# tencent-ailab/pika

Hardware: NVIDIA H100
Metric: utterances/sec RNN-T train step (T=1000,U=150,V=6k) (higher is better)
Workload: dtype bf16

## Files before the change

### pika_b200/csrc/gemm.cu

```cuda
#include <cstdarg>
#include <cstdio>
#include <cstdlib>
#include <cstring>

#include "../../include/pika_b200.h"
#include "common.cuh"

namespace pk {

constexpr int BM = 128;
constexpr int BK = 64;
constexpr int A_STAGE_BYTES = BM * BK * 2;
constexpr int C_STAGE_BYTES = 64 * 128;
constexpr int CONSUMERS = 2;

struct GemmParams {
    CUtensorMap a[PK_GEMM_MAX_PAIRS];
    CUtensorMap b[PK_GEMM_MAX_PAIRS];
    CUtensorMap c;
    int a_off[PK_GEMM_MAX_PAIRS];
    int b_off[PK_GEMM_MAX_PAIRS];
    int n_pairs, kz_count, num_k_blocks;
    int k_splits, iters_per_split;
    int split_major;
    int M, N, tiles_m, tiles_n, zb0, zb1;
    int a_sel2, a_sel3, b_sel2, b_sel3;
    int c_is_f32, c_accumulate;
    float alpha;
    const float* bias;
    int act;
    uint32_t drop_thresh;
    float drop_scale;
    uint32_t drop_seed;
    int aux_mode, aux_is_f32;
    const void* aux;
    long long aux_sm, aux_s0, aux_s1;
    float aux_scale;
    float* row_lse;
    uint64_t pol_a, pol_b, pol_c;
};

template <int BN, bool TWO, bool EPI_WARPS> struct GemmCfg {
    static constexpr int B_STAGE_BYTES = BN * BK * 2;
    static constexpr int STAGE_BYTES = A_STAGE_BYTES + B_STAGE_BYTES;
    static constexpr int STAGES = BN == 256 ? (EPI_WARPS ? 3 : 4) : (BN == 128 ? 6 : 8);
    static constexpr int C_OFF = STAGES * STAGE_BYTES;
    static constexpr int C_BYTES = EPI_WARPS ? BM * BN * 2 : CONSUMERS * 2 * C_STAGE_BYTES;
    static constexpr int BIAS_OFF = C_OFF + C_BYTES;
    static constexpr int BAR_OFF = BIAS_OFF + (EPI_WARPS ? BN * 4 : 0);
    static constexpr int SMEM_BYTES = BAR_OFF + 256 + 1024;
    static constexpr int THREADS = 128 + CONSUMERS * 128;
    static constexpr int RELEASES = CONSUMERS * (TWO ? 2 : 1);
    static_assert(!TWO || BN == 256, "the CTA-pair kernel works on 256 x 256 tiles");
    static_assert(SMEM_BYTES <= 232448, "shared memory budget");
};

PK_DEVICE int pick_sel(int sel, int zb0, int zb1, int kz) {
    return sel == PK_SEL_ZB0 ? zb0 : (sel == PK_SEL_ZB1 ? zb1 : (sel == PK_SEL_KZ ? kz : 0));
}

struct UnitCoord { int mb, nb, zb0, zb1, split; };
PK_DEVICE UnitCoord decode_unit(const GemmParams& p, int unit, int out_tiles) {
    UnitCoord u;
    int tile;
    if (p.split_major) { u.split = unit / out_tiles; tile = unit - u.split * out_tiles; }
    else { tile = unit / p.k_splits; u.split = unit - tile * p.k_splits; }
    const int tiles_per_z = p.tiles_m * p.tiles_n;
    const int z = tile / tiles_per_z;
    const int r = tile - z * tiles_per_z;
    u.mb = r / p.tiles_n; u.nb = r - u.mb * p.tiles_n;
    u.zb1 = z / p.zb0; u.zb0 = z - u.zb1 * p.zb0;
    return u;
}

template <int BN, bool A_MN, bool B_MN> PK_DEVICE void wgmma_tile(float (&acc)[BN / 2], uint64_t a, uint64_t b, uint32_t accumulate) {
    if constexpr (BN == 64) wgmma_ss_n64<A_MN, B_MN>(acc, a, b, accumulate);
    else if constexpr (BN == 128) wgmma_ss_n128<A_MN, B_MN>(acc, a, b, accumulate);
    else wgmma_ss_n256<A_MN, B_MN>(acc, a, b, accumulate);
}

enum { EPI_PLAIN = 0, EPI_LSE = 1, EPI_FULL = 2 };
template <bool CF32, int EPI> constexpr bool epi_warps() { return !CF32 && EPI != EPI_FULL; }

template <bool A_MN, bool B_MN, int BN, bool CF32, int EPI, bool TWO>
__global__ void __launch_bounds__(GemmCfg<BN, TWO, epi_warps<CF32, EPI>()>::THREADS, 1) gemm_wgmma_kernel(const __grid_constant__ GemmParams p) {
    constexpr bool EW = epi_warps<CF32, EPI>();
    static_assert(EPI != EPI_LSE || (EW && BN == 256), "the row log-sum-exp epilogue works on bf16 256-wide tiles");
    using Cfg = GemmCfg<BN, TWO, EW>;
    extern __shared__ uint8_t smem_raw[];
    uint8_t* smem = reinterpret_cast<uint8_t*>((reinterpret_cast<uintptr_t>(smem_raw) + 1023) & ~uintptr_t(1023));
    uint64_t* full_bar = reinterpret_cast<uint64_t*>(smem + Cfg::BAR_OFF);
    uint64_t* empty_bar = full_bar + Cfg::STAGES;
    uint64_t* c_full = empty_bar + Cfg::STAGES;
    uint64_t* c_empty = c_full + 1;
    const uint32_t ctile = smem_u32(smem + Cfg::C_OFF);
    const uint32_t sbias = smem_u32(smem + Cfg::BIAS_OFF);

    const int warp = threadIdx.x >> 5;
    const int lane = threadIdx.x & 31;
    const uint32_t rank = TWO ? cluster_ctarank() : 0u;
    const int worker = TWO ? (int)(blockIdx.x >> 1) : (int)blockIdx.x;
    const int n_workers = TWO ? (int)(gridDim.x >> 1) : (int)gridDim.x;

    if (threadIdx.x == 0) {
        for (int i = 0; i < p.n_pairs; ++i) {
            tma_prefetch_desc(&p.a[i]);
            tma_prefetch_desc(&p.b[i]);
        }
        tma_prefetch_desc(&p.c);
        for (int s = 0; s < Cfg::STAGES; ++s) {
            mbar_init(&full_bar[s], 1);
            mbar_init(&empty_bar[s], Cfg::RELEASES);
        }
        if (EW) {
            mbar_init(c_full, CONSUMERS * 4);
            mbar_init(c_empty, 3);
        }
        mbar_fence_init();
    }
    if (TWO) cluster_sync_all(); else __syncthreads();

    const int out_tiles = p.tiles_m * p.tiles_n * p.zb0 * p.zb1;
    const int num_units = out_tiles * p.k_splits;
    const int k_iters_total = p.n_pairs * p.kz_count * p.num_k_blocks;

    if (warp < 4) {
        setmaxnreg_dec<40>();
    }
    if (warp == 0) {
        const uint32_t lead = elect_one_u32();
        int stage = 0;
        uint32_t phase = 0;
        const int kzb = p.kz_count * p.num_k_blocks;
        for (int unit = worker; unit < num_units; unit += n_workers) {
            const UnitCoord u = decode_unit(p, unit, out_tiles);
            const int m0 = TWO ? u.mb * (2 * BM) + (int)rank * BM : u.mb * BM, n0 = u.nb * BN;
            const int i0 = u.split * p.iters_per_split, i1 = min(k_iters_total, i0 + p.iters_per_split);
            int pr = i0 / kzb;
            int rem = i0 - pr * kzb;
            int kz = rem / p.num_k_blocks, kb = rem - kz * p.num_k_blocks;
            int a2 = pick_sel(p.a_sel2, u.zb0, u.zb1, kz), a3 = pick_sel(p.a_sel3, u.zb0, u.zb1, kz);
            int b2 = pick_sel(p.b_sel2, u.zb0, u.zb1, kz), b3 = pick_sel(p.b_sel3, u.zb0, u.zb1, kz);
            const CUtensorMap* ma = &p.a[pr];
            const CUtensorMap* mbp = &p.b[pr];
            int a_off = p.a_off[pr], b_off = p.b_off[pr];
            for (int i = i0; i < i1; ++i) {
                mbar_wait(&empty_bar[stage], phase ^ 1);
                uint8_t* sa = smem + stage * Cfg::STAGE_BYTES;
                uint8_t* sb = sa + A_STAGE_BYTES;
                mbar_arrive_expect_tx_p(&full_bar[stage], Cfg::STAGE_BYTES, lead);
                const int k0 = kb * BK;
                if (A_MN) {
#pragma unroll
                    for (int c = 0; c < BM / 64; ++c)
                        tma_load_4d_hint_p(sa + c * (64 * BK * 2), ma, &full_bar[stage], m0 + c * 64, k0 + a_off, a2, a3, p.pol_a, lead);
                } else {
                    tma_load_4d_hint_p(sa, ma, &full_bar[stage], k0, m0 + a_off, a2, a3, p.pol_a, lead);
                }
                if (TWO) {
                    if (B_MN) {
#pragma unroll
                        for (int c = 0; c < BN / 128; ++c) {
                            const int cc = (int)rank * (BN / 128) + c;
                            tma_load_4d_mc_hint_p(sb + cc * (64 * BK * 2), mbp, &full_bar[stage], n0 + cc * 64, k0 + b_off, b2, b3, 3, p.pol_b, lead);
                        }
                    } else {
                        tma_load_4d_mc_hint_p(sb + (int)rank * (BN / 2) * 128, mbp, &full_bar[stage], k0, n0 + (int)rank * (BN / 2) + b_off, b2, b3, 3,
                                              p.pol_b, lead);
                    }
                } else if (B_MN) {
#pragma unroll
                    for (int c = 0; c < BN / 64; ++c)
                        tma_load_4d_hint_p(sb + c * (64 * BK * 2), mbp, &full_bar[stage], n0 + c * 64, k0 + b_off, b2, b3, p.pol_b, lead);
                } else {
                    tma_load_4d_hint_p(sb, mbp, &full_bar[stage], k0, n0 + b_off, b2, b3, p.pol_b, lead);
                }
                if (++stage == Cfg::STAGES) { stage = 0; phase ^= 1; }
                if (++kb == p.num_k_blocks) {
                    kb = 0;
                    if (++kz == p.kz_count) {
                        kz = 0;
                        if (++pr < p.n_pairs) { ma = &p.a[pr]; mbp = &p.b[pr]; a_off = p.a_off[pr]; b_off = p.b_off[pr]; }
                    }
                    a2 = pick_sel(p.a_sel2, u.zb0, u.zb1, kz); a3 = pick_sel(p.a_sel3, u.zb0, u.zb1, kz);
                    b2 = pick_sel(p.b_sel2, u.zb0, u.zb1, kz); b3 = pick_sel(p.b_sel3, u.zb0, u.zb1, kz);
                }
            }
        }
    }
    if (EW && warp >= 1 && warp < 4) {
        const int et = threadIdx.x - 32;
        const uint32_t store_pred = (threadIdx.x == 32) ? 1u : 0u;
        uint32_t cph = 0;
        for (int unit = worker; unit < num_units; unit += n_workers, cph ^= 1) {
            const UnitCoord u = decode_unit(p, unit, out_tiles);
            const int m0 = TWO ? u.mb * (2 * BM) + (int)rank * BM : u.mb * BM, n0 = u.nb * BN;
            for (int c = et; c < BN; c += 96) sts_f32(sbias + c * 4, (p.bias != nullptr && n0 + c < p.N) ? __ldg(p.bias + n0 + c) : 0.f);
            __syncwarp();
            if (lane == 0) mbar_arrive(c_empty);
            mbar_wait(c_full, cph);
#pragma unroll
            for (int ch = 0; ch < BN / 64; ++ch)
#pragma unroll
                for (int h = 0; h < 2; ++h)
                    if (n0 + ch * 64 < p.N && m0 + h * 64 < p.M)
                        tma_store_4d_hint_p(&p.c, smem + Cfg::C_OFF + ch * (BM * 128) + h * (64 * 128), n0 + ch * 64, m0 + h * 64, u.zb0, u.zb1,
                                            p.pol_c, store_pred);
            tma_store_commit_p(store_pred);
            if constexpr (EPI == EPI_LSE) {
                constexpr float L2E = 1.4426950408889634f;
                const int half = lane & 1;
                const int nvalid = p.N - n0 - half * 128;
                const int rot = half * 4;
                for (int r = (et >> 5) * 16 + (lane >> 1); r < BM; r += 48) {
                    const uint32_t rowa = ctile + half * (2 * BM * 128) + r * 128;
                    uint32_t mx[4] = {0xFF80FF80u, 0xFF80FF80u, 0xFF80FF80u, 0xFF80FF80u};
#pragma unroll
                    for (int j = 0; j < 16; ++j) {
                        const int g = (j & 7) ^ rot;
                        if ((j >> 3) * 64 + g * 8 < nvalid) {
                            const uint4 v = lds_u32x4(rowa + (j >> 3) * (BM * 128) + ((g ^ (r & 7)) << 4));
                            mx[0] = bf16x2_max(mx[0], v.x); mx[1] = bf16x2_max(mx[1], v.y);
                            mx[2] = bf16x2_max(mx[2], v.z); mx[3] = bf16x2_max(mx[3], v.w);
                        }
                    }
                    const uint32_t m2 = bf16x2_max(bf16x2_max(mx[0], mx[1]), bf16x2_max(mx[2], mx[3]));
                    const float m = fmaxf(bf16lo(m2), bf16hi(m2)) * L2E;
                    float s[4] = {0.f, 0.f, 0.f, 0.f};
#pragma unroll
                    for (int j = 0; j < 16; ++j) {
                        const int g = (j & 7) ^ rot;
                        if ((j >> 3) * 64 + g * 8 < nvalid) {
                            const uint4 v = lds_u32x4(rowa + (j >> 3) * (BM * 128) + ((g ^ (r & 7)) << 4));
                            const uint32_t w[4] = {v.x, v.y, v.z, v.w};
#pragma unroll
                            for (int q = 0; q < 4; ++q)
                                s[q] += ex2_approx(fmaf(bf16lo(w[q]), L2E, -m)) + ex2_approx(fmaf(bf16hi(w[q]), L2E, -m));
                        }
                    }
                    const float sum = (s[0] + s[1]) + (s[2] + s[3]);
                    const float mo = __shfl_xor_sync(0xffffffffu, m, 1);
                    const float so = __shfl_xor_sync(0xffffffffu, sum, 1);
                    const float mm = fmaxf(m, mo);
                    const float st = (mm == -INFINITY) ? 0.f : sum * ex2_approx(m - mm) + so * ex2_approx(mo - mm);
                    if (half == 0 && m0 + r < p.M)
                        *reinterpret_cast<float2*>(p.row_lse + ((size_t)u.nb * (size_t)p.M + (size_t)(m0 + r)) * 2) = make_float2(mm, st);
                }
            }
            tma_store_wait_read_p<0>(store_pred);
        }
        if (store_pred) tma_store_wait<0>();
    }
    if (warp >= 4) {
    setmaxnreg_inc<232>();
    const int wg = (threadIdx.x >> 7) - 1;
    const int et = threadIdx.x & 127;
    const int w4 = et >> 5;
    const uint32_t store_pred = (et == 0) ? 1u : 0u;
    const int bar_stage = 1 + wg;
    constexpr int GW = CF32 ? 4 : 8;
    constexpr int CH = 8 * GW;
    constexpr int ES = CF32 ? 4 : 2;
    uint8_t* cst = smem + Cfg::C_OFF + wg * 2 * C_STAGE_BYTES;
    const float relu_floor = (p.act == PK_ACT_RELU) ? 0.f : -INFINITY;
    const uint32_t base16 = (smem_u32(smem) >> 4) & 0x3FFF;
    const uint64_t a_desc0 = (A_MN ? make_smem_desc_sw128(0, 64 * BK * 2, 1024) : make_smem_desc_sw128(0, 16, 1024)) + base16 + ((wg * 8192) >> 4);
    const uint64_t b_desc0 = (B_MN ? make_smem_desc_sw128(0, 64 * BK * 2, 1024) : make_smem_desc_sw128(0, 16, 1024)) + base16 + (A_STAGE_BYTES >> 4);
    constexpr uint32_t A_K16 = (A_MN ? 2048 : 32) >> 4, B_K16 = (B_MN ? 2048 : 32) >> 4;
    const int r0 = w4 * 16 + (lane >> 2);
    const int cq = (lane & 3) * 2;

    float acc[BN / 2];
    int stage = 0;
    uint32_t phase = 0;
    uint32_t chunk_ctr = 0;
    uint32_t cph = 0;
    auto release = [&](int s) {
        if (et == 0) { mbar_arrive(&empty_bar[s]); if (TWO) mbar_arrive_remote(&empty_bar[s], rank ^ 1u); }
    };
    for (int unit = worker; unit < num_units; unit += n_workers) {
        const UnitCoord u = decode_unit(p, unit, out_tiles);
        const int k_iters = min(k_iters_total, (u.split + 1) * p.iters_per_split) - u.split * p.iters_per_split;
        int prev = -1;
        for (int k = 0; k < k_iters; ++k) {
            mbar_wait(&full_bar[stage], phase);
            const uint32_t st16 = (uint32_t)(stage * Cfg::STAGE_BYTES) >> 4;
            wgmma_fence_acc(acc);
            wgmma_fence();
#pragma unroll
            for (int k4 = 0; k4 < BK / 16; ++k4)
                wgmma_tile<BN, A_MN, B_MN>(acc, a_desc0 + st16 + k4 * A_K16, b_desc0 + st16 + k4 * B_K16, (k > 0 || k4 > 0) ? 1u : 0u);
            wgmma_commit();
            wgmma_fence_acc(acc);
            wgmma_wait<1>();
            if (prev >= 0) release(prev);
            prev = stage;
            if (++stage == Cfg::STAGES) { stage = 0; phase ^= 1; }
        }
        wgmma_wait<0>();
        wgmma_fence_acc(acc);
        if (prev >= 0) release(prev);

        if constexpr (EW) {
            mbar_wait(c_empty, cph);
            const int mi = lane >> 3;
            const uint32_t row_addr = ctile + (uint32_t)(wg * 64 + w4 * 16 + (lane & 7) + ((mi & 1) << 3)) * 128;
#pragma unroll
            for (int q = 0; q < BN / 16; ++q) {
                uint32_t r[4];
#pragma unroll
                for (int i = 0; i < 2; ++i) {
                    const int blk = 2 * q + i;
                    const float2 bs = lds_f32x2(sbias + (blk * 8 + cq) * 4);
#pragma unroll
                    for (int h = 0; h < 2; ++h)
                        r[2 * i + h] = pack_bf16x2(fmaxf(fmaf(acc[blk * 4 + 2 * h], p.alpha, bs.x), relu_floor),
                                                   fmaxf(fmaf(acc[blk * 4 + 2 * h + 1], p.alpha, bs.y), relu_floor));
                }
                const int blk = 2 * q + (mi >> 1);
                stmatrix_x4(row_addr + (blk >> 3) * (BM * 128) + (((blk & 7) ^ (lane & 7)) << 4), r[0], r[1], r[2], r[3]);
            }
            fence_proxy_async_smem();
            __syncwarp();
            if (lane == 0) mbar_arrive(c_full);
            cph ^= 1;
            continue;
        }

        const int zb0 = u.zb0, zb1 = u.zb1;
        const int m0 = (TWO ? u.mb * (2 * BM) + (int)rank * BM : u.mb * BM) + wg * 64;
        const int n0 = u.nb * BN;
        if (m0 >= p.M) continue;
        const int mrow[2] = {m0 + r0, m0 + r0 + 8};
        const unsigned char* aux_row[2] = {nullptr, nullptr};
        uint64_t lin_row[2];
#pragma unroll
        for (int h = 0; h < 2; ++h) {
            if (EPI == EPI_FULL && p.aux_mode != PK_AUX_NONE && mrow[h] < p.M) {
                const long long off = (long long)mrow[h] * p.aux_sm + (long long)zb0 * p.aux_s0 + (long long)zb1 * p.aux_s1;
                aux_row[h] = reinterpret_cast<const unsigned char*>(p.aux) + off * (p.aux_is_f32 ? 4 : 2);
            }
            lin_row[h] = ((uint64_t)(zb1 * p.zb0 + zb0) * (uint64_t)p.M + (uint64_t)mrow[h]) * (uint64_t)p.N;
        }
        constexpr int n_chunks = BN / CH;
#pragma unroll
        for (int ch = 0; ch < n_chunks; ++ch) {
            const int nc0 = n0 + ch * CH;
            if (nc0 >= p.N) break;
            uint8_t* sbuf = cst + (chunk_ctr & 1) * C_STAGE_BYTES;
            tma_store_wait_read_p<1>(store_pred);
            named_bar_sync(bar_stage, 128);
#pragma unroll
            for (int nb = 0; nb < CH / 8; ++nb) {
                const int cl = nb * 8 + cq;
                const int ncol = nc0 + cl;
                float bs[2];
                if (p.bias != nullptr && ncol < p.N) { bs[0] = __ldg(p.bias + ncol); bs[1] = (ncol + 1 < p.N) ? __ldg(p.bias + ncol + 1) : 0.f; }
                else { bs[0] = 0.f; bs[1] = 0.f; }
#pragma unroll
                for (int h = 0; h < 2; ++h) {
                    const int ai = (ch * (CH / 8) + nb) * 4 + 2 * h;
                    float x[2];
#pragma unroll
                    for (int e = 0; e < 2; ++e) x[e] = fmaxf(fmaf(acc[ai + e], p.alpha, bs[e]), relu_floor);
                    if (EPI == EPI_FULL && p.drop_thresh != 0u) {
#pragma unroll
                        for (int e = 0; e < 2; ++e)
                            x[e] = drop_keep(lin_row[h] + (uint64_t)(ncol + e), p.drop_seed, p.drop_thresh) ? x[e] * p.drop_scale : 0.f;
                    }
                    if (EPI == EPI_FULL && aux_row[h] != nullptr && ncol < p.N) {
                        float a[2];
                        if (p.aux_is_f32) {
                            const float2 t2 = *reinterpret_cast<const float2*>(aux_row[h] + (size_t)ncol * 4);
                            a[0] = t2.x; a[1] = t2.y;
                        } else {
                            const uint32_t t1 = *reinterpret_cast<const uint32_t*>(aux_row[h] + (size_t)ncol * 2);
                            a[0] = bf16lo(t1); a[1] = bf16hi(t1);
                        }
                        if (p.aux_mode == PK_AUX_ADD) { x[0] += a[0]; x[1] += a[1]; }
                        else { x[0] = (a[0] != 0.f) ? x[0] * p.aux_scale : 0.f; x[1] = (a[1] != 0.f) ? x[1] * p.aux_scale : 0.f; }
                    }
                    const int row = r0 + 8 * h;
                    const int boff = cl * ES;
                    uint8_t* dst = sbuf + row * 128 + ((((boff >> 4) ^ (row & 7))) << 4) + (boff & 15);
                    if (CF32) {
                        *reinterpret_cast<float2*>(dst) = make_float2(x[0], x[1]);
                    } else {
                        *reinterpret_cast<uint32_t*>(dst) = pack_bf16x2(x[0], x[1]);
                    }
                }
            }
            fence_proxy_async_smem();
            named_bar_sync(bar_stage, 128);
            if (p.c_accumulate) tma_reduce_add_4d_p(&p.c, sbuf, nc0, m0, zb0, zb1, store_pred);
            else tma_store_4d_hint_p(&p.c, sbuf, nc0, m0, zb0, zb1, p.pol_c, store_pred);
            tma_store_commit_p(store_pred);
            ++chunk_ctr;
        }
    }
    if (!EW && store_pred) tma_store_wait<0>();
    }
    if (TWO) cluster_sync_all();
}

typedef CUresult (*EncodeTiledFn)(CUtensorMap*, CUtensorMapDataType, cuuint32_t, void*, const cuuint64_t*,
                                  const cuuint64_t*, const cuuint32_t*, const cuuint32_t*, CUtensorMapInterleave,
                                  CUtensorMapSwizzle, CUtensorMapL2promotion, CUtensorMapFloatOOBfill);

static EncodeTiledFn get_encode_fn() {
    static EncodeTiledFn fn = nullptr;
    if (fn) return fn;
    void* ptr = nullptr;
    cudaDriverEntryPointQueryResult qres;
    cudaError_t e = cudaGetDriverEntryPoint("cuTensorMapEncodeTiled", &ptr, cudaEnableDefault, &qres);
    if (e != cudaSuccess || qres != cudaDriverEntryPointSuccess || ptr == nullptr) return nullptr;
    fn = reinterpret_cast<EncodeTiledFn>(ptr);
    return fn;
}

static int make_map(CUtensorMap* out, const pk_view4& v, int is_f32, int box0, int box1, const char* what) {
    EncodeTiledFn enc = get_encode_fn();
    if (!enc) { set_last_error("cuTensorMapEncodeTiled entry point not available"); return -3; }
    const int es = is_f32 ? 4 : 2;
    cuuint64_t dims[4];
    cuuint64_t strides[3];
    cuuint32_t box[4] = {(cuuint32_t)box0, (cuuint32_t)box1, 1, 1};
    cuuint32_t estr[4] = {1, 1, 1, 1};
    for (int i = 0; i < 4; ++i) {
        if (v.dim[i] <= 0) { set_last_error("gemm %s: dim[%d]=%lld must be > 0", what, i, (long long)v.dim[i]); return -1; }
        dims[i] = (cuuint64_t)v.dim[i];
    }
    for (int i = 0; i < 3; ++i) {
        long long sb = (long long)v.stride[i] * es;
        if (v.dim[i + 1] == 1 && (sb <= 0 || (sb % 16) != 0)) sb = 16;
        if (sb <= 0 || (sb % 16) != 0) {
            set_last_error("gemm %s: stride[%d]=%lld elements is not a positive multiple of 16 bytes", what, i,
                           (long long)v.stride[i]);
            return -1;
        }
        strides[i] = (cuuint64_t)sb;
    }
    if ((reinterpret_cast<uintptr_t>(v.ptr) & 15) != 0) { set_last_error("gemm %s: base pointer not 16B aligned", what); return -1; }
    if ((cuuint64_t)box[1] > 256) { set_last_error("gemm %s: box too large", what); return -1; }
    CUresult r = enc(out, is_f32 ? CU_TENSOR_MAP_DATA_TYPE_FLOAT32 : CU_TENSOR_MAP_DATA_TYPE_BFLOAT16, 4,
                     const_cast<void*>(v.ptr), dims, strides, box, estr, CU_TENSOR_MAP_INTERLEAVE_NONE,
                     CU_TENSOR_MAP_SWIZZLE_128B, CU_TENSOR_MAP_L2_PROMOTION_L2_256B, CU_TENSOR_MAP_FLOAT_OOB_FILL_NONE);
    if (r != CUDA_SUCCESS) { set_last_error("gemm %s: cuTensorMapEncodeTiled failed with CUresult %d", what, (int)r); return -3; }
    return 0;
}

void count_launch();

int encode_tiled_bf16_3d(CUtensorMap* out, const void* ptr, const unsigned long long (&dims)[3], const unsigned long long (&strides_bytes)[2],
                         const unsigned (&box)[3], const char* what) {
    EncodeTiledFn enc = get_encode_fn();
    if (!enc) { set_last_error("cuTensorMapEncodeTiled entry point not available"); return -3; }
    {
        static thread_local bool ctx_ready = false;
        if (!ctx_ready) { PK_CHECK_CUDA(cudaFree(nullptr)); ctx_ready = true; }
    }
    cuuint64_t d[3] = {dims[0], dims[1], dims[2]};
    cuuint64_t st[2] = {strides_bytes[0], strides_bytes[1]};
    cuuint32_t bx[3] = {box[0], box[1], box[2]};
    cuuint32_t es[3] = {1, 1, 1};
    if ((reinterpret_cast<uintptr_t>(ptr) & 15) != 0 || (st[0] % 16) != 0 || (st[1] % 16) != 0) {
        set_last_error("%s: base pointer / strides must be 16-byte aligned", what);
        return -1;
    }
    CUresult r = enc(out, CU_TENSOR_MAP_DATA_TYPE_BFLOAT16, 3, const_cast<void*>(ptr), d, st, bx, es, CU_TENSOR_MAP_INTERLEAVE_NONE,
                     CU_TENSOR_MAP_SWIZZLE_128B, CU_TENSOR_MAP_L2_PROMOTION_L2_256B, CU_TENSOR_MAP_FLOAT_OOB_FILL_NONE);
    if (r != CUDA_SUCCESS) { set_last_error("%s: cuTensorMapEncodeTiled failed with CUresult %d", what, (int)r); return -3; }
    return 0;
}

template <bool A_MN, bool B_MN, int BN, bool CF32, int EPI, bool TWO>
static int launch_gemm_e(const GemmParams& gp, int workers, cudaStream_t stream) {
    using Cfg = GemmCfg<BN, TWO, epi_warps<CF32, EPI>()>;
    auto kern = gemm_wgmma_kernel<A_MN, B_MN, BN, CF32, EPI, TWO>;
    static bool configured = false;
    if (!configured) {
        PK_CHECK_CUDA(cudaFuncSetAttribute(kern, cudaFuncAttributeMaxDynamicSharedMemorySize, Cfg::SMEM_BYTES));
        configured = true;
    }
    if (TWO) {
        cudaLaunchConfig_t cfg = {};
        cfg.gridDim = dim3(2 * workers);
        cfg.blockDim = dim3(Cfg::THREADS);
        cfg.dynamicSmemBytes = Cfg::SMEM_BYTES;
        cfg.stream = stream;
        cudaLaunchAttribute attr[1];
        attr[0].id = cudaLaunchAttributeClusterDimension;
        attr[0].val.clusterDim.x = 2; attr[0].val.clusterDim.y = 1; attr[0].val.clusterDim.z = 1;
        cfg.attrs = attr;
        cfg.numAttrs = 1;
        static int max_pairs = -1;
        if (max_pairs < 0) {
            int n = 0;
            PK_CHECK_CUDA(cudaOccupancyMaxActiveClusters(&n, kern, &cfg));
            PK_CHECK_ARG(n > 0, "gemm: no 2-CTA cluster of the pair kernel fits on this device");
            max_pairs = n;
        }
        if (workers > max_pairs) {
            workers = max_pairs;
            cfg.gridDim = dim3(2 * workers);
        }
        PK_CHECK_CUDA(cudaLaunchKernelEx(&cfg, kern, gp));
    } else {
        kern<<<workers, Cfg::THREADS, Cfg::SMEM_BYTES, stream>>>(gp);
        PK_CHECK_LAUNCH();
    }
    count_launch();
    return 0;
}

template <bool A_MN, bool B_MN, int BN, bool CF32, bool TWO>
static int launch_gemm(const GemmParams& gp, int workers, cudaStream_t stream) {
    if (gp.row_lse != nullptr) {
        if constexpr (!A_MN && !B_MN && BN == 256 && !CF32) return launch_gemm_e<false, false, 256, false, EPI_LSE, TWO>(gp, workers, stream);
        set_last_error("gemm: row_lse needs K-major operands, a bf16 C and block_n = 256");
        return -1;
    }
    if (gp.drop_thresh != 0u || gp.aux_mode != PK_AUX_NONE) return launch_gemm_e<A_MN, B_MN, BN, CF32, EPI_FULL, TWO>(gp, workers, stream);
    return launch_gemm_e<A_MN, B_MN, BN, CF32, EPI_PLAIN, TWO>(gp, workers, stream);
}

template <int BN, bool TWO>
static int dispatch_major(const GemmParams& gp, int a_mn, int b_mn, int workers, cudaStream_t stream) {
    if (gp.c_is_f32) {
        if (!a_mn && !b_mn) return launch_gemm<false, false, BN, true, TWO>(gp, workers, stream);
        if (!a_mn && b_mn) return launch_gemm<false, true, BN, true, TWO>(gp, workers, stream);
        if (a_mn && !b_mn) return launch_gemm<true, false, BN, true, TWO>(gp, workers, stream);
        return launch_gemm<true, true, BN, true, TWO>(gp, workers, stream);
    }
    if (!a_mn && !b_mn) return launch_gemm<false, false, BN, false, TWO>(gp, workers, stream);
    if (!a_mn && b_mn) return launch_gemm<false, true, BN, false, TWO>(gp, workers, stream);
    if (a_mn && !b_mn) return launch_gemm<true, false, BN, false, TWO>(gp, workers, stream);
    return launch_gemm<true, true, BN, false, TWO>(gp, workers, stream);
}

static int env_int(const char* name, int dflt) {
    const char* e = getenv(name);
    return e ? atoi(e) : dflt;
}
static uint64_t policy_of(int code) { return code == 1 ? kL2EvictFirst : (code == 2 ? kL2EvictLast : kL2EvictNormal); }

struct GemmPlan { int bn; bool two; };
static GemmPlan plan_gemm(long long M, long long N, int block_n, int two_sm_req) {
    GemmPlan pl;
    pl.bn = block_n ? block_n : (N <= 64 ? 64 : (N <= 128 ? 128 : 256));
    static int use_2sm = -1;
    if (use_2sm < 0) use_2sm = env_int("PK_GEMM_2SM", 0);
    static int min_tiles = -1;
    if (min_tiles < 0) min_tiles = env_int("PK_GEMM_2SM_MIN_TILES", 1);
    const long long tiles2 = ((M + 255) / 256) * ((N + 255) / 256);
    const int want = two_sm_req < 0 ? 0 : (two_sm_req > 0 ? 1 : (use_2sm && tiles2 >= min_tiles));
    pl.two = want && pl.bn == 256 && M > 128;
    return pl;
}

}

extern "C" int pk_gemm_row_lse_parts(long long M, long long N, int block_n, int two_sm) {
    const pk::GemmPlan pl = pk::plan_gemm(M, N, block_n ? block_n : 256, two_sm);
    return (int)((N + pl.bn - 1) / pl.bn);
}

extern "C" int pk_gemm_bf16(const pk_gemm_desc* d, void* stream_v) {
    using namespace pk;
    cudaStream_t stream = reinterpret_cast<cudaStream_t>(stream_v);
    PK_CHECK_ARG(d != nullptr, "null descriptor");
    PK_CHECK_ARG(d->n_pairs >= 1 && d->n_pairs <= PK_GEMM_MAX_PAIRS, "n_pairs out of range");
    PK_CHECK_ARG(d->kz_count >= 1, "kz_count must be >= 1");
    PK_CHECK_ARG(d->c_dtype == PK_F32 || d->c_dtype == PK_BF16, "bad c_dtype");
    PK_CHECK_ARG(!d->c_accumulate || d->c_dtype == PK_F32, "c_accumulate needs an f32 C");
    PK_CHECK_ARG(d->drop_p >= 0.f && d->drop_p < 1.f, "drop_p out of range");
    const long long N = d->c.dim[0], M = d->c.dim[1];
    PK_CHECK_ARG(M > 0 && N > 0, "empty C");
    PK_CHECK_ARG(d->aux == nullptr || d->aux_mode == PK_AUX_NONE || (N % 8 == 0), "aux epilogue needs N % 8 == 0");
    PK_CHECK_ARG(d->block_n == 0 || d->block_n == 64 || d->block_n == 128 || d->block_n == 256, "block_n must be 64, 128 or 256");
    const GemmPlan plan = plan_gemm(M, N, d->row_lse ? (d->block_n ? d->block_n : 256) : d->block_n, d->two_sm);
    const int bn = plan.bn;
    const bool two_sm = plan.two;

    {
        static thread_local bool ctx_ready = false;
        if (!ctx_ready) { PK_CHECK_CUDA(cudaFree(nullptr)); ctx_ready = true; }
    }
    static thread_local GemmParams gp;
    memset(&gp, 0, sizeof(gp));
    long long K = d->a_mn_major ? d->a[0].dim[1] : d->a[0].dim[0];
    for (int i = 0; i < d->n_pairs; ++i) {
        const long long ka = d->a_mn_major ? d->a[i].dim[1] : d->a[i].dim[0];
        const long long kb = d->b_mn_major ? d->b[i].dim[1] : d->b[i].dim[0];
        PK_CHECK_ARG(ka == K && kb == K, "all pairs must share the reduction extent K");
        int rc = make_map(&gp.a[i], d->a[i], 0, 64, d->a_mn_major ? 64 : BM, "A");
        if (rc) return rc;
        rc = make_map(&gp.b[i], d->b[i], 0, 64, d->b_mn_major ? 64 : (two_sm ? bn / 2 : bn), "B");
        if (rc) return rc;
        gp.a_off[i] = d->a_row_off[i];
        gp.b_off[i] = d->b_row_off[i];
    }
    {
        int rc = make_map(&gp.c, d->c, d->c_dtype == PK_F32, d->c_dtype == PK_F32 ? 32 : 64, 64, "C");
        if (rc) return rc;
    }
    gp.n_pairs = d->n_pairs;
    gp.kz_count = d->kz_count;
    gp.num_k_blocks = (int)((K + BK - 1) / BK);
    gp.M = (int)M;
    gp.N = (int)N;
    gp.tiles_m = (int)(two_sm ? (M + 2 * BM - 1) / (2 * BM) : (M + BM - 1) / BM);
    gp.tiles_n = (int)((N + bn - 1) / bn);
    gp.zb0 = (int)d->c.dim[2];
    gp.zb1 = (int)d->c.dim[3];
    gp.a_sel2 = d->a_sel2; gp.a_sel3 = d->a_sel3; gp.b_sel2 = d->b_sel2; gp.b_sel3 = d->b_sel3;
    gp.c_is_f32 = d->c_dtype == PK_F32;
    gp.c_accumulate = d->c_accumulate;
    gp.alpha = d->alpha;
    gp.bias = d->bias;
    gp.act = d->act;
    if (d->drop_p > 0.f) {
        double t = (double)d->drop_p * 4294967296.0;
        gp.drop_thresh = t >= 4294967295.0 ? 4294967295u : (uint32_t)t;
        if (gp.drop_thresh == 0) gp.drop_thresh = 1;
        gp.drop_scale = 1.f / (1.f - d->drop_p);
    }
    gp.drop_seed = d->drop_seed;
    gp.aux_mode = d->aux ? d->aux_mode : PK_AUX_NONE;
    gp.aux_is_f32 = d->aux_dtype == PK_F32;
    gp.aux = d->aux;
    gp.aux_sm = d->aux_stride[0]; gp.aux_s0 = d->aux_stride[1]; gp.aux_s1 = d->aux_stride[2];
    gp.aux_scale = d->aux_scale;
    gp.row_lse = d->row_lse;
    PK_CHECK_ARG(d->row_lse == nullptr || (d->c_dtype == PK_BF16 && N % 8 == 0 && gp.zb0 == 1 && gp.zb1 == 1 && bn == 256 &&
                                           gp.drop_thresh == 0u && gp.aux_mode == PK_AUX_NONE),
                 "row_lse needs a 2-D bf16 C with N % 8 == 0, block_n = 256, no dropout / aux");
    {
        static int hints = -1;
        if (hints < 0) hints = env_int("PK_GEMM_L2_HINTS", 1);
        const long long K_ = (long long)gp.num_k_blocks * BK * gp.kz_count;
        const long long a_bytes = M * K_ * 2 * gp.n_pairs, b_bytes = N * K_ * 2 * gp.n_pairs;
        const long long c_bytes = M * N * (gp.c_is_f32 ? 4 : 2) * gp.zb0 * gp.zb1;
        const long long small = 32ll << 20, big = 256ll << 20;
        gp.pol_a = policy_of(hints && a_bytes <= small && gp.zb0 * gp.zb1 == 1 ? 2 : 0);
        gp.pol_b = policy_of(hints && b_bytes <= small && gp.zb0 * gp.zb1 == 1 ? 2 : 0);
        gp.pol_c = policy_of(hints && c_bytes >= big ? 1 : 0);
    }

    const long long out_tiles = (long long)gp.tiles_m * gp.tiles_n * gp.zb0 * gp.zb1;
    const int workers_max = two_sm ? num_sms() / 2 : num_sms();
    const int k_iters_total = gp.n_pairs * gp.kz_count * gp.num_k_blocks;
    int splits = 1;
    const bool plain_epi = d->bias == nullptr && d->act == PK_ACT_NONE && d->drop_p == 0.f && gp.aux_mode == PK_AUX_NONE;
    if (d->k_splits > 0) splits = d->k_splits;
    else if (gp.c_is_f32 && plain_epi && gp.zb0 == 1 && gp.zb1 == 1 && k_iters_total >= 16) {
        static int mode = -1, smax = -1;
        if (mode < 0) { mode = env_int("PK_GEMM_SPLIT_MODE", 1); smax = env_int("PK_GEMM_SPLIT_MAX", 16); }
        const int w = workers_max;
        if (mode == 0) {
            if (out_tiles < 2 * w) {
                splits = (int)((2 * w + out_tiles / 2) / out_tiles);
                if (splits > k_iters_total / 8) splits = k_iters_total / 8;
                if (splits > 64) splits = 64;
            }
        } else if (out_tiles < 6 * w) {
            double best = 0.0;
            for (int sp = 1; sp <= smax && sp <= k_iters_total / 8; ++sp) {
                const long long units = out_tiles * sp;
                const double eff = (double)units / (double)(((units + w - 1) / w) * w);
                if (eff > best + 0.02) { best = eff; splits = sp; }
            }
        }
        if (splits < 1) splits = 1;
    }
    PK_CHECK_ARG(splits == 1 || (gp.c_is_f32 && plain_epi && gp.zb0 == 1 && gp.zb1 == 1), "split-K needs a plain f32 2-D C");
    {
        static int sm = -1;
        if (sm < 0) sm = env_int("PK_GEMM_SPLIT_MAJOR", 1);
        gp.split_major = sm;
    }
    gp.iters_per_split = (k_iters_total + splits - 1) / splits;
    gp.k_splits = (k_iters_total + gp.iters_per_split - 1) / gp.iters_per_split;
    if (gp.k_splits > 1) {
        if (!gp.c_accumulate)
            PK_CHECK_CUDA(cudaMemset2DAsync(const_cast<void*>(d->c.ptr), (size_t)d->c.stride[0] * 4, 0, (size_t)N * 4, (size_t)M, stream));
        gp.c_accumulate = 1;
    }
    const long long num_tiles = out_tiles * gp.k_splits;
    PK_CHECK_ARG(num_tiles < (1ll << 31), "too many tiles");
    int grid = workers_max;
    if (num_tiles < grid) grid = (int)num_tiles;
    if (two_sm) return dispatch_major<256, true>(gp, d->a_mn_major, d->b_mn_major, grid, stream);
    if (bn == 64) return dispatch_major<64, false>(gp, d->a_mn_major, d->b_mn_major, grid, stream);
    if (bn == 128) return dispatch_major<128, false>(gp, d->a_mn_major, d->b_mn_major, grid, stream);
    return dispatch_major<256, false>(gp, d->a_mn_major, d->b_mn_major, grid, stream);
}
```

Measured before the change: 180.7.

## Move LSE epilogue into consumer warpgroups, overlapping sum-exp with next tile's mainloop

```diff
diff --git a/pika_b200/csrc/gemm.cu b/pika_b200/csrc/gemm.cu
--- a/pika_b200/csrc/gemm.cu
+++ b/pika_b200/csrc/gemm.cu
@@ -207,46 +207,6 @@
                         tma_store_4d_hint_p(&p.c, smem + Cfg::C_OFF + ch * (BM * 128) + h * (64 * 128), n0 + ch * 64, m0 + h * 64, u.zb0, u.zb1,
                                             p.pol_c, store_pred);
             tma_store_commit_p(store_pred);
-            if constexpr (EPI == EPI_LSE) {
-                constexpr float L2E = 1.4426950408889634f;
-                const int half = lane & 1;
-                const int nvalid = p.N - n0 - half * 128;
-                const int rot = half * 4;
-                for (int r = (et >> 5) * 16 + (lane >> 1); r < BM; r += 48) {
-                    const uint32_t rowa = ctile + half * (2 * BM * 128) + r * 128;
-                    uint32_t mx[4] = {0xFF80FF80u, 0xFF80FF80u, 0xFF80FF80u, 0xFF80FF80u};
-#pragma unroll
-                    for (int j = 0; j < 16; ++j) {
-                        const int g = (j & 7) ^ rot;
-                        if ((j >> 3) * 64 + g * 8 < nvalid) {
-                            const uint4 v = lds_u32x4(rowa + (j >> 3) * (BM * 128) + ((g ^ (r & 7)) << 4));
-                            mx[0] = bf16x2_max(mx[0], v.x); mx[1] = bf16x2_max(mx[1], v.y);
-                            mx[2] = bf16x2_max(mx[2], v.z); mx[3] = bf16x2_max(mx[3], v.w);
-                        }
-                    }
-                    const uint32_t m2 = bf16x2_max(bf16x2_max(mx[0], mx[1]), bf16x2_max(mx[2], mx[3]));
-                    const float m = fmaxf(bf16lo(m2), bf16hi(m2)) * L2E;
-                    float s[4] = {0.f, 0.f, 0.f, 0.f};
-#pragma unroll
-                    for (int j = 0; j < 16; ++j) {
-                        const int g = (j & 7) ^ rot;
-                        if ((j >> 3) * 64 + g * 8 < nvalid) {
-                            const uint4 v = lds_u32x4(rowa + (j >> 3) * (BM * 128) + ((g ^ (r & 7)) << 4));
-                            const uint32_t w[4] = {v.x, v.y, v.z, v.w};
-#pragma unroll
-                            for (int q = 0; q < 4; ++q)
-                                s[q] += ex2_approx(fmaf(bf16lo(w[q]), L2E, -m)) + ex2_approx(fmaf(bf16hi(w[q]), L2E, -m));
-                        }
-                    }
-                    const float sum = (s[0] + s[1]) + (s[2] + s[3]);
-                    const float mo = __shfl_xor_sync(0xffffffffu, m, 1);
-                    const float so = __shfl_xor_sync(0xffffffffu, sum, 1);
-                    const float mm = fmaxf(m, mo);
-                    const float st = (mm == -INFINITY) ? 0.f : sum * ex2_approx(m - mm) + so * ex2_approx(mo - mm);
-                    if (half == 0 && m0 + r < p.M)
-                        *reinterpret_cast<float2*>(p.row_lse + ((size_t)u.nb * (size_t)p.M + (size_t)(m0 + r)) * 2) = make_float2(mm, st);
-                }
-            }
             tma_store_wait_read_p<0>(store_pred);
         }
         if (store_pred) tma_store_wait<0>();
@@ -278,6 +238,36 @@
     auto release = [&](int s) {
         if (et == 0) { mbar_arrive(&empty_bar[s]); if (TWO) mbar_arrive_remote(&empty_bar[s], rank ^ 1u); }
     };
+    constexpr float L2E = 1.4426950408889634f;
+    constexpr int LSE_SLICES = BN / 16;
+    bool lse_pending = false;
+    float lse_m0 = 0.f, lse_m1 = 0.f, lse_s0 = 0.f, lse_s1 = 0.f;
+    int lse_row = 0, lse_nb = 0, lse_nvalid = 0;
+    const uint32_t lse_addr = ctile + (uint32_t)(wg * 64 + r0) * 128;
+    auto lse_slice = [&](int t) {
+        const int j = (t >> 1) & 3, g = (lane & 3) * 2 + (t & 1);
+        if (j * 64 + g * 8 < lse_nvalid) {
+            const bool hi = (t >> 3) != 0;
+            const uint4 v = lds_u32x4(lse_addr + (hi ? 8 * 128 : 0) + j * (BM * 128) + ((g ^ (lane >> 2)) << 4));
+            const float nm = hi ? -lse_m1 : -lse_m0;
+            const uint32_t w[4] = {v.x, v.y, v.z, v.w};
+            float s = 0.f;
+#pragma unroll
+            for (int q = 0; q < 4; ++q) s += ex2_approx(fmaf(bf16lo(w[q]), L2E, nm)) + ex2_approx(fmaf(bf16hi(w[q]), L2E, nm));
+            if (hi) lse_s1 += s; else lse_s0 += s;
+        }
+    };
+    auto lse_finish = [&]() {
+        lse_s0 += __shfl_xor_sync(0xffffffffu, lse_s0, 1);
+        lse_s1 += __shfl_xor_sync(0xffffffffu, lse_s1, 1);
+        lse_s0 += __shfl_xor_sync(0xffffffffu, lse_s0, 2);
+        lse_s1 += __shfl_xor_sync(0xffffffffu, lse_s1, 2);
+        float* dst = p.row_lse + ((size_t)lse_nb * (size_t)p.M + (size_t)lse_row) * 2;
+        if ((lane & 3) == 0 && lse_row < p.M) *reinterpret_cast<float2*>(dst) = make_float2(lse_m0, lse_m0 == -INFINITY ? 0.f : lse_s0);
+        if ((lane & 3) == 0 && lse_row + 8 < p.M)
+            *reinterpret_cast<float2*>(dst + 16) = make_float2(lse_m1, lse_m1 == -INFINITY ? 0.f : lse_s1);
+        lse_pending = false;
+    };
     for (int unit = worker; unit < num_units; unit += n_workers) {
         const UnitCoord u = decode_unit(p, unit, out_tiles);
         const int k_iters = min(k_iters_total, (u.split + 1) * p.iters_per_split) - u.split * p.iters_per_split;
@@ -294,6 +284,9 @@
             wgmma_fence_acc(acc);
             wgmma_wait<1>();
             if (prev >= 0) release(prev);
+            if constexpr (EPI == EPI_LSE) {
+                if (lse_pending && k < LSE_SLICES) lse_slice(k);
+            }
             prev = stage;
             if (++stage == Cfg::STAGES) { stage = 0; phase ^= 1; }
         }
@@ -302,7 +295,16 @@
         if (prev >= 0) release(prev);
 
         if constexpr (EW) {
+            if constexpr (EPI == EPI_LSE) {
+                if (lse_pending) {
+                    for (int t = k_iters; t < LSE_SLICES; ++t) lse_slice(t);
+                    lse_finish();
+                }
+            }
             mbar_wait(c_empty, cph);
+            if constexpr (EPI == EPI_LSE) __syncwarp();
+            const int nvalid = p.N - u.nb * BN;
+            uint32_t mx[2] = {0xFF80FF80u, 0xFF80FF80u};
             const int mi = lane >> 3;
             const uint32_t row_addr = ctile + (uint32_t)(wg * 64 + w4 * 16 + (lane & 7) + ((mi & 1) << 3)) * 128;
 #pragma unroll
@@ -316,6 +318,7 @@
                     for (int h = 0; h < 2; ++h)
                         r[2 * i + h] = pack_bf16x2(fmaxf(fmaf(acc[blk * 4 + 2 * h], p.alpha, bs.x), relu_floor),
                                                    fmaxf(fmaf(acc[blk * 4 + 2 * h + 1], p.alpha, bs.y), relu_floor));
+                    if (EPI == EPI_LSE && blk * 8 < nvalid) { mx[0] = bf16x2_max(mx[0], r[2 * i]); mx[1] = bf16x2_max(mx[1], r[2 * i + 1]); }
                 }
                 const int blk = 2 * q + (mi >> 1);
                 stmatrix_x4(row_addr + (blk >> 3) * (BM * 128) + (((blk & 7) ^ (lane & 7)) << 4), r[0], r[1], r[2], r[3]);
@@ -324,6 +327,19 @@
             __syncwarp();
             if (lane == 0) mbar_arrive(c_full);
             cph ^= 1;
+            if constexpr (EPI == EPI_LSE) {
+                float x0 = fmaxf(bf16lo(mx[0]), bf16hi(mx[0])), x1 = fmaxf(bf16lo(mx[1]), bf16hi(mx[1]));
+                x0 = fmaxf(x0, __shfl_xor_sync(0xffffffffu, x0, 1));
+                x1 = fmaxf(x1, __shfl_xor_sync(0xffffffffu, x1, 1));
+                x0 = fmaxf(x0, __shfl_xor_sync(0xffffffffu, x0, 2));
+                x1 = fmaxf(x1, __shfl_xor_sync(0xffffffffu, x1, 2));
+                lse_m0 = x0 * L2E; lse_m1 = x1 * L2E;
+                lse_s0 = 0.f; lse_s1 = 0.f;
+                lse_row = (TWO ? u.mb * (2 * BM) + (int)rank * BM : u.mb * BM) + wg * 64 + r0;
+                lse_nb = u.nb;
+                lse_nvalid = nvalid;
+                lse_pending = true;
+            }
             continue;
         }
 
@@ -398,6 +414,13 @@
             ++chunk_ctr;
         }
     }
+    if constexpr (EPI == EPI_LSE) {
+        if (lse_pending) {
+#pragma unroll
+            for (int t = 0; t < LSE_SLICES; ++t) lse_slice(t);
+            lse_finish();
+        }
+    }
     if (!EW && store_pred) tma_store_wait<0>();
     }
     if (TWO) cluster_sync_all();
```

Measured after the change: 186.5 (median of 6 runs). +3.2%, better.
